# native-m/whitebox

Hardware: AMD Instinct MI355X
Metric: stereo fp32 frames/sec mixed (4096 tracks @ 512-frame blocks) (higher is better)
Workload: dtype f32

## Files before the change

whitebox_amd/csrc/wbx_mix.h:

```cpp
#pragma once
#include <hip/hip_runtime.h>
#include <hip/hip_ext.h>

#include <cstdlib>
#include <type_traits>

#include "wbx_dev.h"
#include "wbx_shape.h"

namespace wbx {

typedef float f4 __attribute__((ext_vector_type(4)));
typedef float f4u __attribute__((ext_vector_type(4), aligned(4)));

#define WBX_GLOBAL __attribute__((address_space(1)))
template <class T>
__device__ __forceinline__ const T WBX_GLOBAL* as_global(const void* p) {
  return (const T WBX_GLOBAL*)(uintptr_t)p;
}

__device__ __forceinline__ void store_f4_system(float* p, f4 v) {
  asm volatile("global_store_dwordx4 %0, %1, off sc0 sc1" : : "v"(p), "v"(v) : "memory");
}
__device__ __forceinline__ void store_u4_system(void* p, uint4 u) {
  const f4 v = {__uint_as_float(u.x), __uint_as_float(u.y), __uint_as_float(u.z), __uint_as_float(u.w)};
  asm volatile("global_store_dwordx4 %0, %1, off sc0 sc1" : : "v"(p), "v"(v) : "memory");
}

__device__ __forceinline__ float clampf(float x, float lo, float hi) {
  float m = x < hi ? x : hi;
  return m > lo ? m : lo;
}
__device__ __forceinline__ double clampd(double x, double lo, double hi) {
  double m = x < hi ? x : hi;
  return m > lo ? m : lo;
}

__device__ __forceinline__ float absmax4(f4 m) {
  float t;
  asm("v_max3_f32 %0, |%1|, |%2|, |%3|" : "=v"(t) : "v"(m.x), "v"(m.y), "v"(m.z));
  asm("v_max_f32_e64 %0, |%1|, %2" : "=v"(t) : "v"(m.w), "v"(t));
  return t;
}

__device__ __forceinline__ float sel_neg(int t, float a, float b) {
  const int m = t >> 31;
  float r;
  asm("v_bfi_b32 %0, %1, %2, %3" : "=v"(r) : "v"(m), "v"(a), "v"(b));
  return r;
}
template <int E>
__device__ __forceinline__ void taps(const f4& v, float w4, int k, float& sa, float& sb) {
  sa = v.x;
  sb = v.y;
  if (E >= 1) {
    sa = sel_neg(k - 1, sa, v.y);
    sb = sel_neg(k - 1, sb, v.z);
  }
  if (E >= 2) {
    sa = sel_neg(k - 2, sa, v.z);
    sb = sel_neg(k - 2, sb, v.w);
  }
  if (E >= 3) {
    sa = sel_neg(k - 3, sa, v.w);
    sb = sel_neg(k - 3, sb, w4);
  }
}

constexpr double kNarrowSpeed = 0.67;
template <int E>
__device__ __forceinline__ void taps_narrow(const f4& v, float w4, int k, float& sa, float& sb) {
  const int t = k - E;
  if (E == 1) {
    sa = sel_neg(t, v.x, v.y);
    sb = sel_neg(t, v.y, v.z);
  } else if (E == 2) {
    sa = sel_neg(t, v.y, v.z);
    sb = sel_neg(t, v.z, v.w);
  } else {
    sa = sel_neg(t, v.z, v.w);
    sb = sel_neg(t, v.w, w4);
  }
}

__device__ __forceinline__ float wave_max_lane63(float x) {
  uint32_t v = __float_as_uint(x);
#define WBX_DPP_MAX(ctrl, rmask)                                                                      \
  {                                                                                                  \
    const uint32_t o = (uint32_t)__builtin_amdgcn_update_dpp(0, (int)v, (ctrl), (rmask), 0xF, true);  \
    v = v > o ? v : o;                                                                               \
  }
  WBX_DPP_MAX(0xB1, 0xF)
  WBX_DPP_MAX(0x4E, 0xF)
  WBX_DPP_MAX(0x141, 0xF)
  WBX_DPP_MAX(0x140, 0xF)
  WBX_DPP_MAX(0x142, 0xA)
  WBX_DPP_MAX(0x143, 0xC)
#undef WBX_DPP_MAX
  return __uint_as_float(v);
}

__device__ __forceinline__ uint32_t wave_max_quad(uint32_t p0, uint32_t p1, uint32_t p2, uint32_t p3) {
  typedef unsigned int u2v __attribute__((ext_vector_type(2)));
  const u2v a = __builtin_amdgcn_permlane32_swap(p0, p1, false, false);
  const uint32_t m01 = a.x > a.y ? a.x : a.y;
  const u2v b = __builtin_amdgcn_permlane32_swap(p2, p3, false, false);
  const uint32_t m23 = b.x > b.y ? b.x : b.y;
  const u2v c = __builtin_amdgcn_permlane16_swap(m01, m23, false, false);
  uint32_t v = c.x > c.y ? c.x : c.y;
#define WBX_DPP_MAX(ctrl)                                                                         \
  {                                                                                               \
    const uint32_t o = (uint32_t)__builtin_amdgcn_update_dpp(0, (int)v, (ctrl), 0xF, 0xF, true);  \
    v = v > o ? v : o;                                                                            \
  }
  WBX_DPP_MAX(0xB1) WBX_DPP_MAX(0x4E) WBX_DPP_MAX(0x141) WBX_DPP_MAX(0x140)
#undef WBX_DPP_MAX
  return v;
}

__device__ __forceinline__ void wave_max_quad_halves(uint32_t p0, uint32_t p1, uint32_t p2, uint32_t p3, uint32_t& ch0,
                                                     uint32_t& ch1) {
  typedef unsigned int u2v __attribute__((ext_vector_type(2)));
  const u2v a = __builtin_amdgcn_permlane32_swap(p0, p1, false, false);
  const u2v b = __builtin_amdgcn_permlane32_swap(p2, p3, false, false);
  const u2v c0 = __builtin_amdgcn_permlane16_swap(a.x, b.x, false, false);
  const u2v c1 = __builtin_amdgcn_permlane16_swap(a.y, b.y, false, false);
  uint32_t v = c0.x > c0.y ? c0.x : c0.y, w = c1.x > c1.y ? c1.x : c1.y;
#define WBX_DPP_MAX(x, ctrl)                                                                      \
  {                                                                                               \
    const uint32_t o = (uint32_t)__builtin_amdgcn_update_dpp(0, (int)(x), (ctrl), 0xF, 0xF, true); \
    (x) = (x) > o ? (x) : o;                                                                      \
  }
  WBX_DPP_MAX(v, 0xB1) WBX_DPP_MAX(v, 0x4E) WBX_DPP_MAX(v, 0x141) WBX_DPP_MAX(v, 0x140)
  WBX_DPP_MAX(w, 0xB1) WBX_DPP_MAX(w, 0x4E) WBX_DPP_MAX(w, 0x141) WBX_DPP_MAX(w, 0x140)
#undef WBX_DPP_MAX
  ch0 = v;
  ch1 = w;
}

enum : int { MODE_U = 0, MODE_W = 1, MODE_I16 = 2, MODE_I32 = 3, MODE_MIXED = 4, MODE_WN = 5, MODE_G = 6, MODE_WI = 7, MODE_WIN = 8, MODE_MU = 9, MODE_MW = 10, MODE_MWN = 11,
             MODE_WNU = 12, MODE_WINU = 13 };

struct Win {
  f4 v;
  float w4;
};
template <int CL>
struct PreT {
  Win w[CL];
  int ix0;
  float fx0;
};
template <int CL>
struct PreGT {
  f4 v[CL], b[CL], fx;
};
template <int CL>
struct RowT {
  f4 c[CL];
};

template <int U, bool FULL, int FAM, int SB, int CW, int CL, int T, int X = 0>
__device__ __forceinline__ void mix_body(const MixArgs& a) {
  constexpr bool G = FAM == 1 || FAM == 3;
  constexpr bool STRIDE = FAM == 1;
  constexpr bool W16 = FAM >= 1;
  constexpr bool LEAN16 = FAM == 2;
  static_assert(SB == 1 || FULL, "sub-blocks need waves that stay inside one block");
  static_assert(CW == 1 || (CW == 2 && (SB == 4 || (SB == 1 && T == 64))), "two channels per wave: 128-frame stereo blocks, one block per wave");
  static_assert(CL == 1 || (CL == 2 && FULL && SB == 1 && CW == 1), "two channels per lane: stereo blocks of 4 * T frames");
  static_assert(T == 256 / CL || (CL == 2 && (T == 64 || T == 256)) || (CL == 1 && SB == 1 && (T == 64 || T == 128)), "lanes per workgroup");
  constexpr uint32_t kT = (uint32_t)T;
  constexpr bool XP = X != 0;
  static_assert(!XP || (SB > 1 && FULL), "masked rows in a packed instance");
  constexpr uint32_t kSt = XP ? (kStage >> (X == 1 ? 1 : 0)) / (SB == 4 ? 2u : 1u) : SB == 4 ? kStage / 2 : kT == 64u ? kStage / 2 : kStage;
  constexpr bool EXP = XP || (SB == 1 && FULL && (kSt == 128 || kT == 64u));
  constexpr uint32_t kMaxRows = EXP ? 2 * kSt : kSt;
  constexpr uint32_t kRecs = kMaxRows + 2 * U + 4;
  __shared__ __attribute__((aligned(16))) DTrackBlock s_tb[SB * kRecs];
  constexpr uint32_t kWaves = kT / 64u;
  constexpr uint32_t kPS = (CL == 2 && kWaves == 4u) ? 8u : 4u;
  __shared__ uint32_t s_pk[SB * kRecs * kPS];
  __shared__ uint32_t s_wc[kPS];
  __shared__ __attribute__((aligned(16))) DRow s_rows[EXP ? 2 * SB * kSt : 1];
  __shared__ uint32_t s_ord[EXP ? kSt : 1];
  __shared__ uint16_t s_map[EXP ? SB * 2 * kSt : 1];
  __shared__ uint16_t s_off[EXP ? SB * (kSt + 1) : 1];
  __shared__ uint32_t s_wpairs[3];
  __shared__ uint32_t s_hp[XP ? 8 : 1];
  __shared__ uint32_t s_tot[XP ? SB : 1];
  __shared__ int s_shape;

  const unsigned long long dbg_t0 = a.dbg_clock ? wall_clock64() : 0ull;
  uint32_t bx = blockIdx.x;
  if ((gridDim.x & 7u) == 0u) bx = (blockIdx.x & 7u) * (gridDim.x >> 3) + (blockIdx.x >> 3);
  const uint32_t g = blockIdx.y, tile = blockIdx.z;
  const uint32_t tid = threadIdx.x;
  const DGroup grp = a.groups[g];
  const uint32_t F = a.block_frames, C = a.channels, N = a.n_tracks;
  const uint32_t S4 = F >> 2;
  const uint32_t Lc = FULL ? a.lane_span : S4;
  const uint32_t sub = SB > 1 ? (uint32_t)__builtin_amdgcn_readfirstlane((int)(tid / (C * Lc))) : 0u;
  const uint32_t rb = sub * kRecs;
  const uint32_t b = bx * SB + sub;
  const bool bvalid = SB == 1 || b < a.n_blocks;
  const uint32_t slot = SB > 1 ? tid - sub * (C * Lc) : tile * kT + tid;
  const bool active = FULL ? true : (slot < C * S4);
  uint32_t c = active ? slot / Lc : 0u;
  if (FULL && CL == 1 && c >= C) c = C - 1u;
  if (FULL && CW == 1) c = __builtin_amdgcn_readfirstlane(c);
  const uint32_t jn = active ? slot - (slot / Lc) * Lc : 0u;
  if (CL == 2) c = 0u;
  const bool owns = FULL ? (jn < S4 && slot < C * Lc) : active;
  const uint32_t j0 = active ? (jn < S4 ? jn : S4 - 1u) * 4u : 0u;
  uint32_t span = 64u;
  if (!FULL) {
    span = S4 & (~S4 + 1u);
    span = span > 64u ? 64u : span;
  }
  const uint32_t lane = tid & 63u;
  const double j0d = (double)(int32_t)j0;

  using Pre = PreT<CL>;
  using PreG = PreGT<CL>;
  using Row = RowT<CL>;
  Row acc;
#pragma unroll
  for (int ch = 0; ch < CL; ch++) acc.c[ch] = f4{0.0f, 0.0f, 0.0f, 0.0f};
  if (a.init && g == 0u && owns && bvalid) {
#pragma unroll
    for (int ch = 0; ch < CL; ch++)
      acc.c[ch] = *reinterpret_cast<const f4*>(a.init + ((size_t)b * C + (CL == 2 ? (uint32_t)ch : c)) * F + j0);
  }

  const bool chain_in = a.chain != nullptr && (grp.flags & GROUP_CHAIN_IN) != 0u;
  const bool chain_out = a.chain != nullptr && (grp.flags & GROUP_CHAIN_OUT) != 0u;
  uint32_t* chain_word = a.chain ? a.chain + ((size_t)(blockIdx.x * a.tiles + tile) * a.n_groups + g) : nullptr;
  const uint32_t my_xcc = a.chain ? ((uint32_t)__builtin_amdgcn_s_getreg(63508) & 0xFu) + 1u : 0u;
  const uint32_t chain_tag = a.chain_epoch << 4;
  uint32_t chain_seen = 0u;
  if (chain_in && tid == 0u) chain_seen = __hip_atomic_load(chain_word - 1, __ATOMIC_RELAXED, __HIP_MEMORY_SCOPE_AGENT);

  const double jd1 = j0d + 1.0, jd2 = j0d + 2.0, jd3 = j0d + 3.0;
  const double us = a.uniform_speed;
  const double up0 = __dmul_rn(j0d, us), up1 = __dmul_rn(jd1, us), up2 = __dmul_rn(jd2, us), up3 = __dmul_rn(jd3, us);

  struct URec {
    const void* src[CL];
    double pos, speed;
    float gain, gc[CL];
    uint32_t kind, format;
    uint32_t d, n;
    bool partial;
  };
  auto load_urec = [&](uint32_t rec) {
    const int w = (int)reinterpret_cast<const uint32_t*>(&s_tb[rb + rec])[lane & 15u];
    auto rl = [&](uint32_t i) { return (uint32_t)__builtin_amdgcn_readlane(w, (int)i); };
    URec r;
    if (CW == 2) {
      const uint64_t s0 = ((uint64_t)rl(1) << 32) | rl(0), s1 = ((uint64_t)rl(3) << 32) | rl(2);
      r.src[0] = (const void*)(c ? s1 : s0);
      r.pos = __longlong_as_double((long long)(((uint64_t)rl(5) << 32) | rl(4)));
      r.speed = __longlong_as_double((long long)(((uint64_t)rl(7) << 32) | rl(6)));
      r.gain = __uint_as_float(rl(8));
      r.gc[0] = __uint_as_float(c ? rl(10) : rl(9));
      const uint32_t q11 = rl(11);
      r.kind = (q11 >> 8) & KIND_MASK;
      r.format = rl(13) & 0xFFu;
      if (EXP) {
        r.partial = ((q11 >> 15) & 1u) != 0u;
        r.d = 0u;
        r.n = F;
        if (r.partial) {
          r.d = q11 >> 16;
          r.n = rl(12) & 0xFFFFu;
        }
      }
      return r;
    }
    const uint32_t cs = FULL ? c : 0u;
#pragma unroll
    for (int ch = 0; ch < CL; ch++) {
      const uint32_t cc = CL == 2 ? (uint32_t)ch : cs;
      r.src[ch] = (const void*)(((uint64_t)rl(2u * cc + 1u) << 32) | rl(2u * cc));
      r.gc[ch] = __uint_as_float(rl(9u + cc));
    }
    r.pos = __longlong_as_double((long long)(((uint64_t)rl(5) << 32) | rl(4)));
    r.speed = __longlong_as_double((long long)(((uint64_t)rl(7) << 32) | rl(6)));
    r.gain = __uint_as_float(rl(8));
    const uint32_t q11 = rl(11);
    r.kind = (q11 >> 8) & KIND_MASK;
    r.format = rl(13) & 0xFFu;
    if (EXP) {
      r.partial = ((q11 >> 15) & 1u) != 0u;
      r.d = 0u;
      r.n = F;
      if (r.partial) {
        r.d = q11 >> 16;
        r.n = rl(12) & 0xFFFFu;
      }
    }
    return r;
  };
  const uint32_t wave_base = (uint32_t)__builtin_amdgcn_readfirstlane((int)j0);
  constexpr uint32_t kWF = CW == 2 ? 128u : 256u;
  const uint32_t wave_end = wave_base + kWF < F ? wave_base + kWF : F;
  auto call_frame = [&](uint32_t e, uint32_t d, uint32_t n) {
    const int x = (int)(j0 + e) - (int)d, hi = (int)n - 1;
    const int lo = x > 0 ? x : 0;
    return lo < hi ? lo : hi;
  };
  auto frame_mask = [&](uint32_t e, uint32_t d, uint32_t n) { return (uint32_t)0 - (uint32_t)((j0 + e - d) < n); };
  auto and_mask = [&](float v, uint32_t m) { return __uint_as_float(__float_as_uint(v) & m); };
  auto fast_part = [&](const URec& r) {
    return EXP && a.fast_partial != 0u && r.partial && __double2hiint(r.pos) >= 0x40100000;
  };
  auto part_cf0 = [&](const URec& r) {
    if (fast_part(r)) {
      const int x = (int)j0 - (int)r.d, hi = (int)r.n - 1;
      return ((int)j0 + 3 < (int)r.d) ? 0 : (x < hi ? x : hi);
    }
    return call_frame(0u, r.d, r.n);
  };

  auto row_f32 = [&](const f4& v, float cg, float gc) {
    f4 m;
    if (__float_as_uint(cg) == 0x3F800000u) {
      m.x = __fmul_rn(v.x, gc);
      m.y = __fmul_rn(v.y, gc);
      m.z = __fmul_rn(v.z, gc);
      m.w = __fmul_rn(v.w, gc);
    } else {
      m.x = __fmul_rn(__fmul_rn(v.x, cg), gc);
      m.y = __fmul_rn(__fmul_rn(v.y, cg), gc);
      m.z = __fmul_rn(__fmul_rn(v.z, cg), gc);
      m.w = __fmul_rn(__fmul_rn(v.w, cg), gc);
    }
    return m;
  };
  auto norm_i16 = [&](int lo, int hi) {
    const float norm = 1.0f / 32767.0f;
// ... 567 lines not shown
        const uint32_t fmt = (uint32_t)__builtin_amdgcn_readfirstlane((int)r.format);
        constexpr std::integral_constant<bool, MODE == MODE_MWN> narrow{};
        if (EXP && r.partial) {
          if (r.d >= wave_end || r.d + r.n <= wave_base) {
#pragma unroll
            for (int ch = 0; ch < CL; ch++) m.c[ch] = f4{0.0f, 0.0f, 0.0f, 0.0f};
          } else {
            Pre q = pre[u];
            const bool p16 = k == KIND_WINDOW_I16 || k == KIND_UNITY_I16;
            if (p16) {
#pragma unroll
              for (int ch = 0; ch < CL; ch++) q.w[ch].w4 = pre[u].w[ch].v.z;
            }
            m = partial_any(narrow, q, k, fmt, p16);
          }
        } else if (k == KIND_WINDOW_I16) {
          Pre q = pre[u];
#pragma unroll
          for (int ch = 0; ch < CL; ch++) q.w[ch].w4 = pre[u].w[ch].v.z;
          m = row_window16(narrow, std::false_type{}, q, r.pos, r.speed, cg, gc);
        } else if (k == KIND_WINDOW) {
          if (fmt == FMT_F32)
            m = row_window(narrow, pre[u], r.pos, r.speed, cg, gc);
          else
            m = row_window32(narrow, std::false_type{}, pre[u], fmt, r.pos, r.speed, cg, gc);
        } else if (k == KIND_UNITY_I16) {
          each_i16();
        } else if (k == KIND_UNITY_I32) {
          each_i32(fmt);
        } else {
          each_f32();
        }
      } else {
        const int k = MODE == MODE_U ? KIND_UNITY : MODE == MODE_I16 ? KIND_UNITY_I16 : MODE == MODE_I32 ? KIND_UNITY_I32
                                                  : __builtin_amdgcn_readfirstlane((int)r.kind);
        const uint32_t fmt = (MODE == MODE_I32 || MODE == MODE_MU) ? (uint32_t)__builtin_amdgcn_readfirstlane((int)r.format) : 0u;
        if (EXP && r.partial && !(r.d <= wave_base && r.d + r.n >= wave_end)) {
          if (r.d >= wave_end || r.d + r.n <= wave_base) {
#pragma unroll
            for (int ch = 0; ch < CL; ch++) m.c[ch] = f4{0.0f, 0.0f, 0.0f, 0.0f};
          } else if (fast_part(r)) {
            if (k == KIND_UNITY_I16)
              each_i16();
            else if (k == KIND_UNITY_I32)
              each_i32(fmt);
            else
              each_f32();
            mask_row(m, r.d, r.n);
          } else if (k == KIND_UNITY_I16) {
            each([&](const Win& w, float g) {
              return row_f32_masked(norm_i16(__float_as_int(w.v.x), __float_as_int(w.v.y)), r.d, r.n, cg, g);
            });
          } else if (k == KIND_UNITY_I32) {
            each([&](const Win& w, float g) { return row_f32_masked(norm_i32(w.v, fmt), r.d, r.n, cg, g); });
          } else {
            each([&](const Win& w, float g) { return row_f32_masked(w.v, r.d, r.n, cg, g); });
          }
        } else if (k == KIND_UNITY_I16) {
          each_i16();
        } else if (k == KIND_UNITY_I32) {
          each_i32(fmt);
        } else {
          each_f32();
        }
      }
      }
      add_row(m, pk[u]);
    }
  };

  auto pipeline = [&](auto mode, uint32_t cn) {
    constexpr int D = decltype(mode)::value == MODE_G ? 1 : U;
    constexpr int kIter = (2 * D) % 4 == 0 ? 2 * D : 4;
    std::conditional_t<decltype(mode)::value == MODE_G, PreG, Pre> pa[D], pb[D];
    issue(mode, 0, pa);
    for (uint32_t u0 = 0; u0 < cn; u0 += kIter) {
      float pk[kIter][CL];
#pragma unroll
      for (int h = 0; h < kIter; h += 2 * D) {
        issue(mode, u0 + h + D, pb);
        render(mode, u0 + h, pa, pk + h);
        issue(mode, u0 + h + 2 * D, pa);
        render(mode, u0 + h + D, pb, pk + h + D);
      }
#pragma unroll
      for (int ch = 0; ch < CL; ch++) {
        if (FULL) {
#pragma unroll
          for (int q = 0; q < kIter; q += 4) {
            const float quad[4] = {pk[q][ch], pk[q + 1][ch], pk[q + 2][ch], pk[q + 3][ch]};
            post_peak4(quad, u0 + q, ch);
          }
        } else {
#pragma unroll
          for (int q = 0; q < kIter; q++) post_peak(pk[q][ch], u0 + q, ch);
        }
      }
    }
  };

  auto mixed = [&](uint32_t cn) {
    for (uint32_t tl = 0; tl < cn; tl++) {
      const DTrackBlock& r = s_tb[rb + tl];
      const int k = __builtin_amdgcn_readfirstlane((int)(r.kind & KIND_MASK));
      const float cg = r.gain;
      const uint32_t off = (uint32_t)r.pos + j0;
      Row m;
      float gcs[CL];
      const void* srcs[CL];
#pragma unroll
      for (int ch = 0; ch < CL; ch++) {
        const uint32_t cc = CL == 2 ? (uint32_t)ch : c;
        gcs[ch] = r.g[cc];
        srcs[ch] = r.src[cc];
      }
      if (k == KIND_WINDOW) {
        Pre p;
        load_window(srcs, r.pos, __dmul_rn(j0d, r.speed), p);
        m = row_window(std::false_type{}, p, r.pos, r.speed, cg, gcs);
      } else if (W16 && (k == KIND_WINDOW_I16 || (EXP && LEAN16 && k == KIND_UNITY_I16 && (r.kind & KIND_PARTIAL)))) {
        Pre p;
        if (EXP && LEAN16 && (r.kind & KIND_PARTIAL)) {
          const uint32_t d = r.dst_start, n = r.len;
          load_window16(srcs, r.pos, __dmul_rn((double)call_frame(0u, d, n), r.speed), p);
          m = row_window16_masked(p, r.pos, r.speed, k != KIND_WINDOW_I16, d, n, cg, gcs);
        } else {
          load_window16(srcs, r.pos, __dmul_rn(j0d, r.speed), p);
          m = row_window16(std::false_type{}, std::false_type{}, p, r.pos, r.speed, cg, gcs);
        }
      } else {
#pragma unroll
        for (int ch = 0; ch < CL; ch++) {
          if (k == KIND_UNITY_I16) {
            typedef int i2u __attribute__((ext_vector_type(2), aligned(2)));
            i2u w = {0, 0};
            if (active) w = *reinterpret_cast<const i2u WBX_GLOBAL*>(as_global<short>(srcs[ch]) + off);
            m.c[ch] = row_i16(w.x, w.y, cg, gcs[ch]);
          } else {
            f4 v = {0.0f, 0.0f, 0.0f, 0.0f};
            if (active) v = *reinterpret_cast<const f4u WBX_GLOBAL*>(as_global<float>(srcs[ch]) + off);
            m.c[ch] = (k == KIND_UNITY_I32) ? row_i32(v, r.format, cg, gcs[ch]) : row_f32(v, cg, gcs[ch]);
          }
        }
      }
      float pk[CL];
      add_row(m, pk);
#pragma unroll
      for (int ch = 0; ch < CL; ch++) post_peak(pk[ch], tl, ch);
    }
  };

  uint32_t chunk0 = 0u, cn2 = 0u;
  int mode = MODE_U;
  for (uint32_t chunk_i = 0u; chunk0 < grp.count; chunk_i++) {
    const uint32_t left = grp.count - chunk0;
    const uint32_t cn = left < kSt ? left : kSt;
    cn2 = cn;
    __syncthreads();
    if (tid == 0u) s_shape = 0;
    if constexpr (XP) {
      constexpr uint32_t kHalves = kSt / 32u;
      DRow* rows_cur = s_rows + (chunk_i & 1u) * (SB * kSt);
      DRow* rows_nxt = s_rows + ((chunk_i & 1u) ^ 1u) * (SB * kSt);
      const uint32_t n0 = chunk0 + cn, nleft = grp.count - n0, ncn = nleft < kSt ? nleft : kSt;
      const uint32_t m0 = n0 + ncn, mleft = grp.count - m0, mcn = mleft < kSt ? mleft : kSt;
      uint32_t before = 0u;
      bool is_pair = false;
      const uint32_t psb = tid / kSt, pt = tid - psb * kSt;
      DRow nrow;
      nrow.pos = 0.0;
      nrow.tmpl = 0xFFFFFFFFu;
      nrow.flags = ROW_SILENT;
      uint32_t nord = 0u;
      if (tid < SB * kSt) {
        DRow row = nrow;
        const uint32_t bb = bx * SB + psb;
        const bool bval = bb < a.n_blocks;
        uint32_t o1 = 0u;
        if (chunk_i == 0u) {
          uint32_t o0 = 0u;
          if (pt < cn) o0 = a.order[grp.first + pt];
          if (pt < ncn) o1 = a.order[grp.first + n0 + pt];
          if (pt < cn && bval) row = a.rows[(size_t)bb * N + o0];
          *reinterpret_cast<uint4*>(&rows_cur[tid]) = *reinterpret_cast<const uint4*>(&row);
        } else {
          row = rows_cur[tid];
          o1 = s_ord[pt];
        }
        if (pt < ncn && bval) nrow = a.rows[(size_t)bb * N + o1];
        if (psb == 0u && pt < mcn) nord = a.order[grp.first + m0 + pt];
        is_pair = (row.flags & (ROW_PAIR | ROW_SILENT)) == ROW_PAIR;
        const unsigned long long half = (lane & 32u) ? 0xFFFFFFFF00000000ull : 0x00000000FFFFFFFFull;
        const unsigned long long bal = __ballot(is_pair) & half;
        before = (uint32_t)__popcll(bal & ((1ull << lane) - 1ull));
        if ((lane & 31u) == 0u) s_hp[tid >> 5] = (uint32_t)__popcll(bal);
      }
      __syncthreads();
      if (tid < SB * kSt) {
        uint32_t off = pt + before, total = cn;
#pragma unroll
        for (uint32_t h = 0; h < kHalves; h++) {
          const uint32_t n = s_hp[psb * kHalves + h];
          if (psb * kHalves + h < (tid >> 5)) off += n;
          total += n;
        }
        if (pt < cn) {
          s_off[psb * (kSt + 1u) + pt] = (uint16_t)off;
          s_map[psb * 2u * kSt + off] = (uint16_t)pt;
          if (is_pair) s_map[psb * 2u * kSt + off + 1u] = (uint16_t)(pt | 0x8000u);
        }
        if (pt == 0u) {
          s_off[psb * (kSt + 1u) + cn] = (uint16_t)total;
          s_tot[psb] = total;
        }
      }
      __syncthreads();
      cn2 = (uint32_t)__builtin_amdgcn_readfirstlane((int)s_tot[sub]);
      constexpr uint32_t kQ = (SB * kRecs * 4u + kT - 1u) / kT;
      uint4 wq[kQ];
      uint32_t tq = tid;
      asm volatile("" : "+v"(tq));
#pragma unroll
      for (uint32_t it = 0; it < kQ; it++) {
        const uint32_t i = tq + it * kT, sbq = i / (kRecs * 4u), r4 = i - sbq * (kRecs * 4u), rec = r4 >> 2, q = r4 & 3u;
        const bool in = sbq < (uint32_t)SB && rec < s_tot[sbq < (uint32_t)SB ? sbq : 0u];
        const uint32_t mp = s_map[in ? sbq * 2u * kSt + rec : 0u];
        const DRow row = rows_cur[(in ? sbq * kSt : 0u) + (mp & 0x7FFFu)];
        const bool live = in && !(row.flags & ROW_SILENT);
        wq[it] = reinterpret_cast<const uint4*>(a.tmpl + (live ? row.tmpl + (mp >> 15) : 0u))[q];
      }
#pragma unroll
      for (uint32_t it = 0; it < kQ; it++) {
        const uint32_t i = tq + it * kT, sbq = i / (kRecs * 4u), r4 = i - sbq * (kRecs * 4u), rec = r4 >> 2, q = r4 & 3u;
        if (i < SB * kRecs * 4u) {
          uint4 w = {0u, 0u, 0u, 0u};
          if (rec < s_tot[sbq]) {
            const uint32_t mp = s_map[sbq * 2u * kSt + rec];
            const DRow row = rows_cur[sbq * kSt + (mp & 0x7FFFu)];
            if (!(row.flags & ROW_SILENT)) {
              w = wq[it];
              if (q == 1u && (row.flags & ROW_POS)) {
                const uint2 pb = *reinterpret_cast<const uint2*>(&row.pos);
                w.x = pb.x;
                w.y = pb.y;
              }
            }
          }
          reinterpret_cast<uint4*>(s_tb)[i] = w;
        }
      }
      if (tid < SB * kSt) {
        *reinterpret_cast<uint4*>(&rows_nxt[tid]) = *reinterpret_cast<const uint4*>(&nrow);
        if (psb == 0u) s_ord[pt] = nord;
      }
    } else if constexpr (EXP) {
      DRow* rows_cur = s_rows + (chunk_i & 1u) * kSt;
      DRow* rows_nxt = s_rows + ((chunk_i & 1u) ^ 1u) * kSt;
      const uint32_t n0 = chunk0 + cn, nleft = grp.count - n0, ncn = nleft < kSt ? nleft : kSt;
      const uint32_t m0 = n0 + ncn, mleft = grp.count - m0, mcn = mleft < kSt ? mleft : kSt;
      uint32_t before = 0u;
      bool is_pair = false;
      DRow nrow;
      nrow.pos = 0.0;
      nrow.tmpl = 0xFFFFFFFFu;
      nrow.flags = ROW_SILENT;
      uint32_t nord = 0u;
      if (tid < kSt) {
        DRow row = nrow;
        uint32_t o1 = 0u;
        if (chunk_i == 0u) {
          uint32_t o0 = 0u;
          if (tid < cn) o0 = a.order[grp.first + tid];
          if (tid < ncn) o1 = a.order[grp.first + n0 + tid];
          if (tid < cn) row = a.rows[(size_t)bx * N + o0];
        } else {
          row = rows_cur[tid];
          o1 = s_ord[tid];
        }
        if (tid < ncn) nrow = a.rows[(size_t)bx * N + o1];
        if (tid < mcn) nord = a.order[grp.first + m0 + tid];
        if (chunk_i == 0u) *reinterpret_cast<uint4*>(&rows_cur[tid]) = *reinterpret_cast<const uint4*>(&row);
        is_pair = (row.flags & (ROW_PAIR | ROW_SILENT)) == ROW_PAIR;
        const unsigned long long bal = __ballot(is_pair);
        before = (uint32_t)__popcll(bal & ((1ull << lane) - 1ull));
        if (lane == 0u) s_wpairs[tid >> 6] = (uint32_t)__popcll(bal);
        if (kSt <= 64u && tid == 0u) s_wpairs[1] = 0u;
      }
      __syncthreads();
      if (tid < cn) {
        const uint32_t off = tid + before + (tid >= 64u ? s_wpairs[0] : 0u);
        s_off[tid] = (uint16_t)off;
        s_map[off] = (uint16_t)tid;
        if (is_pair) s_map[off + 1u] = (uint16_t)(tid | 0x8000u);
      }
      if (tid == 0u) {
        const uint32_t total = cn + s_wpairs[0] + s_wpairs[1];
        s_off[cn] = (uint16_t)total;
        s_wpairs[2] = total;
      }
      __syncthreads();
      cn2 = (uint32_t)__builtin_amdgcn_readfirstlane((int)s_wpairs[2]);
      constexpr uint32_t kQ = (kRecs * 4u + kT - 1u) / kT;
      const uint32_t nq = (cn2 * 4u + kT - 1u) / kT;
      uint4 wq[kQ];
      uint32_t tq = tid;
      asm volatile("" : "+v"(tq));
#pragma unroll
      for (uint32_t it = 0; it < kQ; it++) {
        wq[it] = uint4{0u, 0u, 0u, 0u};
        if (it < nq) {
          const uint32_t i = tq + it * kT, rec = i >> 2, q = i & 3u;
          const bool in = rec < cn2;
          const uint32_t mp = s_map[in ? rec : 0u];
          const DRow row = rows_cur[mp & 0x7FFFu];
          const bool live = in && !(row.flags & ROW_SILENT);
          wq[it] = reinterpret_cast<const uint4*>(a.tmpl + (live ? row.tmpl + (mp >> 15) : 0u))[q];
        }
      }
#pragma unroll
      for (uint32_t it = 0; it < kQ; it++) {
        const uint32_t i = tq + it * kT, rec = i >> 2, q = i & 3u;
        if (i < kRecs * 4u) {
          uint4 w = {0u, 0u, 0u, 0u};
          if (it < nq && rec < cn2) {
            const uint32_t mp = s_map[rec];
            const DRow row = rows_cur[mp & 0x7FFFu];
            if (!(row.flags & ROW_SILENT)) {
              w = wq[it];
              if (q == 1u && (row.flags & ROW_POS)) {
                const uint2 pb = *reinterpret_cast<const uint2*>(&row.pos);
                w.x = pb.x;
                w.y = pb.y;
              }
            }
          }
          reinterpret_cast<uint4*>(s_tb)[i] = w;
        }
      }
      if (tid < kSt) {
        *reinterpret_cast<uint4*>(&rows_nxt[tid]) = *reinterpret_cast<const uint4*>(&nrow);
        s_ord[tid] = nord;
      }
    } else {
    for (uint32_t i = tid; i < SB * kRecs * 4u; i += kT) {
      const uint32_t sb = SB > 1 ? i / (kRecs * 4u) : 0u;
      const uint32_t rec = (i - sb * kRecs * 4u) >> 2, q = i & 3u;
      const uint32_t bb = bx * SB + sb;
      uint4 w = {0u, 0u, 0u, 0u};
      if (rec < cn && (SB == 1 || bb < a.n_blocks)) {
        const uint32_t track = a.order[grp.first + chunk0 + rec];
        const DRow row = a.rows[(size_t)bb * N + track];
        if (!(row.flags & ROW_SILENT)) {
          w = reinterpret_cast<const uint4*>(a.tmpl + row.tmpl)[q];
          if (q == 1u && (row.flags & ROW_POS)) {
            const uint2 pb = *reinterpret_cast<const uint2*>(&row.pos);
            w.x = pb.x;
            w.y = pb.y;
          }
        }
      }
      reinterpret_cast<uint4*>(s_tb)[i] = w;
    }
    }
    for (uint32_t i = tid; i < SB * kRecs * kPS; i += kT) s_pk[i] = 0u;
    if (FULL && lane == 0u) {
      if (CL == 2) {
        s_wc[wave] = 0u;
        s_wc[kWaves + wave] = 1u;
        if (2u * kWaves < kPS && wave == 0u) {
          s_wc[2] = 0xFFFFFFFFu;
          s_wc[3] = 0xFFFFFFFFu;
        }
      } else {
        s_wc[wave] = sub * C + c;
      }
    }
    __syncthreads();
    int shape = 0;
    for (uint32_t i0 = tid; i0 < SB * (XP ? kMaxRows : cn2); i0 += kT) {
      if (XP && i0 % kMaxRows >= s_tot[XP ? i0 / kMaxRows : 0u]) continue;
      const uint32_t i = XP ? (i0 / kMaxRows) * kRecs + i0 % kMaxRows : SB > 1 ? (i0 / cn2) * kRecs + i0 % cn2 : i0;
      const int k = s_tb[i].kind & KIND_MASK;
      shape |= k == KIND_UNITY ? 1 : k == KIND_WINDOW ? (s_tb[i].format == FMT_F32 ? 2 : 128) : k == KIND_UNITY_I16 ? 4 : k == KIND_UNITY_I32 ? 8
               : k == KIND_STRIDE ? 64 : k == KIND_WINDOW_I16 ? 32 : 0;
      if ((k == KIND_WINDOW || k == KIND_WINDOW_I16) && !(s_tb[i].speed >= kNarrowSpeed)) shape |= 16;
    }
    if (shape) atomicOr(&s_shape, shape);
    __syncthreads();
    const int shapes = __builtin_amdgcn_readfirstlane(s_shape);
    const int has_f32 = shapes & 3, has_win = shapes & 2, has_i16 = shapes & 4, has_i32 = shapes & 8, has_wide = shapes & 16;
    const int has_stride = STRIDE ? (shapes & 64) : 0;
    const int has_win16 = W16 ? (shapes & 32) : 0;
    const int has_win32 = G ? (shapes & 128) : 0;
    if (LEAN16) {
      if (has_win16)
        mode = (!has_f32 && !has_i32) ? (has_wide ? MODE_WI : us > 0.0 ? MODE_WINU : MODE_WIN) : MODE_MIXED;
      else if (has_i16)
        mode = (!has_f32 && !has_i32) ? MODE_I16 : (has_win || has_i32) ? MODE_MIXED : MODE_MU;
      else
        mode = (has_win || has_i32) ? MODE_MIXED : MODE_U;
    } else if (has_stride) {
      mode = MODE_G;
    } else if (has_win16) {
      mode = (!has_f32 && !has_i32 && !has_win32) ? (has_wide ? MODE_WI : us > 0.0 ? MODE_WINU : MODE_WIN) : (has_wide ? MODE_MW : MODE_MWN);
    } else if (has_i16) {
      mode = (has_win32 || (G && has_win)) ? (has_wide ? MODE_MW : MODE_MWN)
             : (!has_i32 && !has_f32) ? MODE_I16 : has_win ? MODE_MIXED : MODE_MU;
    } else if (has_win || has_win32) {
      mode = (G || !has_i32) ? (has_wide ? MODE_W : us > 0.0 ? MODE_WNU : MODE_WN) : MODE_MIXED;
    } else {
      mode = !has_i32 ? MODE_U : !has_f32 ? MODE_I32 : MODE_MU;
    }
    for (uint32_t i = tid; i < SB * kRecs; i += kT) {
      DTrackBlock& r = s_tb[i];
      if ((SB > 1 ? i % kRecs : i) >= (XP ? s_tot[XP ? i / kRecs : 0u] : cn2) || (r.kind & KIND_MASK) == KIND_SILENT || (r.kind & KIND_MASK) == KIND_GENERIC) {
        r.src[0] = a.zero_page;
        r.src[1] = a.zero_page;
        r.pos = 0.0;
        r.speed = 1.0;
        r.gain = 0.0f;
        r.g[0] = 0.0f;
        r.g[1] = 0.0f;
        r.dst_start = 0;
        r.len = (uint16_t)F;
        const bool m16 = mode == MODE_I16 || mode == MODE_WI || mode == MODE_WIN || mode == MODE_WINU;
        r.format = m16 ? FMT_I16 : mode == MODE_I32 ? FMT_I32 : FMT_F32;
        r.kind = m16 ? KIND_UNITY_I16 : mode == MODE_I32 ? KIND_UNITY_I32 : KIND_UNITY;
      }
    }
    __syncthreads();

    if (chain_in && chunk_i == 0u) {
      if (tid == 0u) {
        uint32_t spins = 0u;
        while ((chain_seen & ~0xFu) != chain_tag && spins < 400000u) {
          __builtin_amdgcn_s_sleep(8);
          chain_seen = __hip_atomic_load(chain_word - 1, __ATOMIC_RELAXED, __HIP_MEMORY_SCOPE_AGENT);
          spins++;
        }
        const bool chain_ok = (chain_seen & ~0xFu) == chain_tag;
        if (!chain_ok && a.chain_status) {
          atomicOr(a.chain_status, 32u);
          atomicOr(a.chain_sticky, 32u);
        }
        if (chain_ok && (chain_seen & 0xFu) != my_xcc && a.chain_status) {
          atomicOr(a.chain_status, 64u);
          atomicOr(a.chain_sticky, 64u);
        }
      }
      __syncthreads();
      if (owns && bvalid) {
#pragma unroll
        for (int ch = 0; ch < CL; ch++) {
          const uint32_t* src = reinterpret_cast<const uint32_t*>(
              a.partial + (((size_t)b * a.n_groups + (g - 1u)) * C + (CL == 2 ? (uint32_t)ch : c)) * F + j0);
          acc.c[ch].x = __uint_as_float(__hip_atomic_load(src + 0, __ATOMIC_RELAXED, __HIP_MEMORY_SCOPE_AGENT));
          acc.c[ch].y = __uint_as_float(__hip_atomic_load(src + 1, __ATOMIC_RELAXED, __HIP_MEMORY_SCOPE_AGENT));
          acc.c[ch].z = __uint_as_float(__hip_atomic_load(src + 2, __ATOMIC_RELAXED, __HIP_MEMORY_SCOPE_AGENT));
          acc.c[ch].w = __uint_as_float(__hip_atomic_load(src + 3, __ATOMIC_RELAXED, __HIP_MEMORY_SCOPE_AGENT));
        }
      }
    }

    switch (mode) {
      case MODE_U: pipeline(std::integral_constant<int, MODE_U>{}, cn2); break;
      case MODE_W:
        if constexpr (!LEAN16) pipeline(std::integral_constant<int, MODE_W>{}, cn2);
        break;
      case MODE_WN:
        if constexpr (!LEAN16) pipeline(std::integral_constant<int, MODE_WN>{}, cn2);
        break;
      case MODE_WNU:
        if constexpr (!LEAN16) pipeline(std::integral_constant<int, MODE_WNU>{}, cn2);
        break;
      case MODE_G:
        if constexpr (STRIDE) pipeline(std::integral_constant<int, MODE_G>{}, cn2);
        break;
      case MODE_WI:
        if constexpr (W16) pipeline(std::integral_constant<int, MODE_WI>{}, cn2);
        break;
      case MODE_WIN:
        if constexpr (W16) pipeline(std::integral_constant<int, MODE_WIN>{}, cn2);
        break;
      case MODE_WINU:
        if constexpr (W16) pipeline(std::integral_constant<int, MODE_WINU>{}, cn2);
        break;
      case MODE_MU: pipeline(std::integral_constant<int, MODE_MU>{}, cn2); break;
      case MODE_MW:
        if constexpr (G) pipeline(std::integral_constant<int, MODE_MW>{}, cn2);
        break;
      case MODE_MWN:
        if constexpr (G) pipeline(std::integral_constant<int, MODE_MWN>{}, cn2);
        break;
      case MODE_I16: pipeline(std::integral_constant<int, MODE_I16>{}, cn2); break;
      case MODE_I32:
        if constexpr (!LEAN16) pipeline(std::integral_constant<int, MODE_I32>{}, cn2);
        break;
      default: mixed(cn2); break;
    }

    __syncthreads();
    for (uint32_t i0 = tid; i0 < SB * cn * C; i0 += kT) {
      const uint32_t sb = SB > 1 ? i0 / (cn * C) : 0u;
      const uint32_t i = i0 - sb * cn * C;
      const uint32_t rec = i / C, ch = i - rec * C;
      const uint32_t bb = bx * SB + sb;
      if (SB > 1 && bb >= a.n_blocks) continue;
      const uint32_t track = a.order[grp.first + chunk0 + rec];
      uint32_t* dst = reinterpret_cast<uint32_t*>(a.peaks) + ((size_t)bb * N + track) * C + ch;
      uint32_t pk = 0u;
      if (FULL && CW == 2) {
        const uint32_t r0 = EXP ? s_off[sb * (kSt + 1u) + rec] : rec;
        const uint32_t r1 = EXP ? s_off[sb * (kSt + 1u) + rec + 1u] : rec + 1u;
        for (uint32_t rr = r0; rr < r1; rr++) {
          const uint32_t v = s_pk[(sb * kRecs + rr) * kPS + ch];
          pk = pk > v ? pk : v;
        }
      } else if (FULL) {
        const uint32_t r0 = EXP ? s_off[sb * (kSt + 1u) + rec] : rec;
        const uint32_t r1 = EXP ? s_off[sb * (kSt + 1u) + rec + 1u] : rec + 1u;
        for (uint32_t rr = r0; rr < r1; rr++) {
          const uint32_t* slots = &s_pk[(sb * kRecs + rr) * kPS];
#pragma unroll
          for (uint32_t w = 0; w < kPS; w++)
            if (s_wc[w] == sb * C + ch) pk = pk > slots[w] ? pk : slots[w];
        }
      } else {
        pk = s_pk[rec * 2u + ch];
      }
      if (a.tiles == 1u)
        *dst = pk;
      else
        atomicMax(dst, pk);
      if (a.levels && pk != 0u) atomicMax(a.levels + (size_t)track * C + ch, pk);
    }
    chunk0 += cn;
  }

  if (a.dbg_clock && tid == 0u) {
    const uint32_t wg = blockIdx.x + gridDim.x * (blockIdx.y + gridDim.y * blockIdx.z);
    a.dbg_clock[4u * wg] = dbg_t0;
    a.dbg_clock[4u * wg + 1u] = wall_clock64();
    a.dbg_clock[4u * wg + 2u] = (unsigned long long)(uint32_t)__builtin_amdgcn_s_getreg(63492);
    a.dbg_clock[4u * wg + 3u] = (unsigned long long)(uint32_t)__builtin_amdgcn_s_getreg(63508);
  }
  if (a.fused_master) {
    if (a.fused_status_dst && blockIdx.x == 0u && tid < 4u) {
      const uint32_t queued = a.fused_status_src[2];
      if (a.partial_through)
        __hip_atomic_store(a.fused_status_dst + tid, a.fused_status_src[tid], __ATOMIC_RELAXED, __HIP_MEMORY_SCOPE_SYSTEM);
      else
        a.fused_status_dst[tid] = a.fused_status_src[tid];
      if (a.fused_zero_status && queued == 0u) a.fused_status_src[tid] = 0u;
    }
    if (owns && bvalid) {
#pragma unroll
      for (int ch = 0; ch < CL; ch++) {
        f4 m = acc.c[ch];
        m.x = __fadd_rn(0.0f, m.x);
        m.y = __fadd_rn(0.0f, m.y);
        m.z = __fadd_rn(0.0f, m.z);
        m.w = __fadd_rn(0.0f, m.w);
        if (a.fused_clamp) {
          m.x = m.x > 1.0f ? 1.0f : (m.x < -1.0f ? -1.0f : m.x);
          m.y = m.y > 1.0f ? 1.0f : (m.y < -1.0f ? -1.0f : m.y);
          m.z = m.z > 1.0f ? 1.0f : (m.z < -1.0f ? -1.0f : m.z);
          m.w = m.w > 1.0f ? 1.0f : (m.w < -1.0f ? -1.0f : m.w);
        }
        float* mo = a.fused_master + ((size_t)b * C + (CL == 2 ? (uint32_t)ch : c)) * F + j0;
        if (a.partial_through)
          store_f4_system(mo, m);
        else
          *reinterpret_cast<f4*>(mo) = m;
      }
    }
  } else if (owns && bvalid) {
#pragma unroll
    for (int ch = 0; ch < CL; ch++) {
      float* out = a.partial + (((size_t)b * a.n_groups + g) * C + (CL == 2 ? (uint32_t)ch : c)) * F + j0;
      if (a.partial_through) {
        uint32_t* o = reinterpret_cast<uint32_t*>(out);
        __hip_atomic_store(o + 0, __float_as_uint(acc.c[ch].x), __ATOMIC_RELAXED, __HIP_MEMORY_SCOPE_AGENT);
        __hip_atomic_store(o + 1, __float_as_uint(acc.c[ch].y), __ATOMIC_RELAXED, __HIP_MEMORY_SCOPE_AGENT);
        __hip_atomic_store(o + 2, __float_as_uint(acc.c[ch].z), __ATOMIC_RELAXED, __HIP_MEMORY_SCOPE_AGENT);
        __hip_atomic_store(o + 3, __float_as_uint(acc.c[ch].w), __ATOMIC_RELAXED, __HIP_MEMORY_SCOPE_AGENT);
      } else {
        *reinterpret_cast<f4*>(out) = acc.c[ch];
      }
    }
  }
  if (chain_out) {
    __builtin_amdgcn_s_waitcnt(0);
    __syncthreads();
    if (tid == 0u) __hip_atomic_store(chain_word, chain_tag | my_xcc, __ATOMIC_RELAXED, __HIP_MEMORY_SCOPE_AGENT);
  }
}

template <int U, bool FULL, int W, int FAM, int SB, int CW = 1, int CL = 1, int T = 256 / CL>
__global__ __launch_bounds__(T, W) void mix_kernel(MixArgs a) {
  mix_body<U, FULL, FAM, SB, CW, CL, T>(a);
}
template <int U, int W, int FAM, int SB, int CW, int X>
__global__ __launch_bounds__(256, W) void mix_kernel_x(MixArgs a) {
  mix_body<U, true, FAM, SB, CW, 1, 256, X>(a);
}

struct MixEntry {
  MixInstance inst;
  const char* name;
  void (*launch)(const MixArgs& a, dim3 grid, hipStream_t s, hipEvent_t t0, hipEvent_t t1);
};
#define WBX_MIX(U, FULL, W, FAM, SB, CW, CL, T)                                                                \
  {MixInstance::mix(U, FULL, W, FAM, SB, CW, CL, T),                                                           \
// ... 32 lines not shown
```

Before: 185.0 million.

## Fold shape detection and zero-row patching into staging pass, trim barriers

Computes the per-record shape bitmask and the zero-row flags while the track records are staged, in registers, using quad DPP broadcasts and a wave OR-reduction. This removes the separate LDS re-scan and its barrier. Zero-row patching now rewrites only flagged quads, the window-pair offset map skips its extra barrier when no pairs exist, s_pk clearing is skipped in FULL mode, and chained partial loads use vectorised dwordx4 agent-scope loads instead of scalar atomics. The cost is more register state and extra DPP/ALU work per staged quad, plus inline asm with explicit waitcnt.

```diff
diff --git a/whitebox_amd/csrc/wbx_mix.h b/whitebox_amd/csrc/wbx_mix.h
--- a/whitebox_amd/csrc/wbx_mix.h
+++ b/whitebox_amd/csrc/wbx_mix.h
@@ -25,6 +25,23 @@
 __device__ __forceinline__ void store_u4_system(void* p, uint4 u) {
   const f4 v = {__uint_as_float(u.x), __uint_as_float(u.y), __uint_as_float(u.z), __uint_as_float(u.w)};
   asm volatile("global_store_dwordx4 %0, %1, off sc0 sc1" : : "v"(p), "v"(v) : "memory");
+}
+
+__device__ __forceinline__ f4 load_f4_agent(const float* p) {
+  f4 v;
+  asm volatile("global_load_dwordx4 %0, %1, off sc1\n\ts_waitcnt vmcnt(0)" : "=&v"(v) : "v"(p) : "memory");
+  return v;
+}
+__device__ __forceinline__ void load_f4x2_agent(const float* p0, const float* p1, f4& v0, f4& v1) {
+  asm volatile("global_load_dwordx4 %0, %2, off sc1\n\tglobal_load_dwordx4 %1, %3, off sc1\n\ts_waitcnt vmcnt(0)"
+               : "=&v"(v0), "=&v"(v1)
+               : "v"(p0), "v"(p1)
+               : "memory");
+}
+
+template <int Q>
+__device__ __forceinline__ uint32_t quad_bcast(uint32_t v) {
+  return (uint32_t)__builtin_amdgcn_update_dpp(0, (int)v, Q * 0x55, 0xF, 0xF, true);
 }
 
 __device__ __forceinline__ float clampf(float x, float lo, float hi) {
@@ -98,6 +115,36 @@
   WBX_DPP_MAX(0x143, 0xC)
 #undef WBX_DPP_MAX
   return __uint_as_float(v);
+}
+
+__device__ __forceinline__ uint32_t wave_or_lane63(uint32_t v) {
+#define WBX_DPP_OR(ctrl, rmask) v |= (uint32_t)__builtin_amdgcn_update_dpp(0, (int)v, (ctrl), (rmask), 0xF, true);
+  WBX_DPP_OR(0xB1, 0xF)
+  WBX_DPP_OR(0x4E, 0xF)
+  WBX_DPP_OR(0x141, 0xF)
+  WBX_DPP_OR(0x140, 0xF)
+  WBX_DPP_OR(0x142, 0xA)
+  WBX_DPP_OR(0x143, 0xC)
+#undef WBX_DPP_OR
+  return v;
+}
+
+__device__ __forceinline__ int staged_record_shape(const uint4& w, bool& zero_row) {
+  const int k = (int)((quad_bcast<2>(w.w) >> 8) & KIND_MASK);
+  const uint32_t format = quad_bcast<3>(w.y) & 0xFFu;
+  const double speed = __hiloint2double((int)quad_bcast<1>(w.w), (int)quad_bcast<1>(w.z));
+  zero_row = k == KIND_SILENT || k == KIND_GENERIC;
+  int shape = k == KIND_UNITY ? 1 : k == KIND_WINDOW ? (format == FMT_F32 ? 2 : 128) : k == KIND_UNITY_I16 ? 4 : k == KIND_UNITY_I32 ? 8
+              : k == KIND_STRIDE ? 64 : k == KIND_WINDOW_I16 ? 32 : 0;
+  if ((k == KIND_WINDOW || k == KIND_WINDOW_I16) && !(speed >= kNarrowSpeed)) shape |= 16;
+  return shape;
+}
+__device__ __forceinline__ uint4 stage_zero_quad(uint4 w, uint32_t q, const void* zero_page, uint32_t F, uint32_t kind, uint32_t format) {
+  const uint32_t zlo = (uint32_t)(uintptr_t)zero_page, zhi = (uint32_t)((uintptr_t)zero_page >> 32);
+  if (q == 0u) return uint4{zlo, zhi, zlo, zhi};
+  if (q == 1u) return uint4{0u, 0u, 0u, 0x3FF00000u};
+  if (q == 2u) return uint4{0u, 0u, 0u, (w.w & 0xFFu) | (kind << 8)};
+  return uint4{(w.x & 0xFFFF0000u) | (F & 0xFFFFu), (w.y & 0xFFFFFF00u) | format, w.z, w.w};
 }
 
 __device__ __forceinline__ uint32_t wave_max_quad(uint32_t p0, uint32_t p1, uint32_t p2, uint32_t p3) {
@@ -186,7 +233,7 @@
   __shared__ uint32_t s_ord[EXP ? kSt : 1];
   __shared__ uint16_t s_map[EXP ? SB * 2 * kSt : 1];
   __shared__ uint16_t s_off[EXP ? SB * (kSt + 1) : 1];
-  __shared__ uint32_t s_wpairs[3];
+  __shared__ uint32_t s_wpairs[2];
   __shared__ uint32_t s_hp[XP ? 8 : 1];
   __shared__ uint32_t s_tot[XP ? SB : 1];
   __shared__ int s_shape;
@@ -1060,12 +1107,14 @@
 
   uint32_t chunk0 = 0u, cn2 = 0u;
   int mode = MODE_U;
+  if (tid == 0u) s_shape = 0;
   for (uint32_t chunk_i = 0u; chunk0 < grp.count; chunk_i++) {
     const uint32_t left = grp.count - chunk0;
     const uint32_t cn = left < kSt ? left : kSt;
     cn2 = cn;
     __syncthreads();
-    if (tid == 0u) s_shape = 0;
+    int shape = 0;
+    uint32_t zero_quads = 0u;
     if constexpr (XP) {
       constexpr uint32_t kHalves = kSt / 32u;
       DRow* rows_cur = s_rows + (chunk_i & 1u) * (SB * kSt);
@@ -1140,21 +1189,24 @@
 #pragma unroll
       for (uint32_t it = 0; it < kQ; it++) {
         const uint32_t i = tq + it * kT, sbq = i / (kRecs * 4u), r4 = i - sbq * (kRecs * 4u), rec = r4 >> 2, q = r4 & 3u;
-        if (i < SB * kRecs * 4u) {
-          uint4 w = {0u, 0u, 0u, 0u};
-          if (rec < s_tot[sbq]) {
-            const uint32_t mp = s_map[sbq * 2u * kSt + rec];
-            const DRow row = rows_cur[sbq * kSt + (mp & 0x7FFFu)];
-            if (!(row.flags & ROW_SILENT)) {
-              w = wq[it];
-              if (q == 1u && (row.flags & ROW_POS)) {
-                const uint2 pb = *reinterpret_cast<const uint2*>(&row.pos);
-                w.x = pb.x;
-                w.y = pb.y;
-              }
+        uint4 w = {0u, 0u, 0u, 0u};
+        if (i < SB * kRecs * 4u && rec < s_tot[sbq]) {
+          const uint32_t mp = s_map[sbq * 2u * kSt + rec];
+          const DRow row = rows_cur[sbq * kSt + (mp & 0x7FFFu)];
+          if (!(row.flags & ROW_SILENT)) {
+            w = wq[it];
+            if (q == 1u && (row.flags & ROW_POS)) {
+              const uint2 pb = *reinterpret_cast<const uint2*>(&row.pos);
+              w.x = pb.x;
+              w.y = pb.y;
             }
           }
+        }
+        bool zero_row;
+        shape |= staged_record_shape(w, zero_row);
+        if (i < SB * kRecs * 4u) {
           reinterpret_cast<uint4*>(s_tb)[i] = w;
+          zero_quads |= (zero_row ? 1u : 0u) << it;
         }
       }
       if (tid < SB * kSt) {
@@ -1193,21 +1245,25 @@
         before = (uint32_t)__popcll(bal & ((1ull << lane) - 1ull));
         if (lane == 0u) s_wpairs[tid >> 6] = (uint32_t)__popcll(bal);
         if (kSt <= 64u && tid == 0u) s_wpairs[1] = 0u;
+        if (tid < cn) {
+          s_off[tid] = (uint16_t)tid;
+          s_map[tid] = (uint16_t)tid;
+        }
+        if (tid == 0u) s_off[cn] = (uint16_t)cn;
       }
       __syncthreads();
-      if (tid < cn) {
-        const uint32_t off = tid + before + (tid >= 64u ? s_wpairs[0] : 0u);
-        s_off[tid] = (uint16_t)off;
-        s_map[off] = (uint16_t)tid;
-        if (is_pair) s_map[off + 1u] = (uint16_t)(tid | 0x8000u);
-      }
-      if (tid == 0u) {
-        const uint32_t total = cn + s_wpairs[0] + s_wpairs[1];
-        s_off[cn] = (uint16_t)total;
-        s_wpairs[2] = total;
-      }
-      __syncthreads();
-      cn2 = (uint32_t)__builtin_amdgcn_readfirstlane((int)s_wpairs[2]);
+      const uint32_t pairs = (uint32_t)__builtin_amdgcn_readfirstlane((int)(s_wpairs[0] + s_wpairs[1]));
+      if (pairs != 0u) {
+        if (tid < cn) {
+          const uint32_t off = tid + before + (tid >= 64u ? s_wpairs[0] : 0u);
+          s_off[tid] = (uint16_t)off;
+          s_map[off] = (uint16_t)tid;
+          if (is_pair) s_map[off + 1u] = (uint16_t)(tid | 0x8000u);
+        }
+        if (tid == 0u) s_off[cn] = (uint16_t)(cn + pairs);
+        __syncthreads();
+      }
+      cn2 = cn + pairs;
       constexpr uint32_t kQ = (kRecs * 4u + kT - 1u) / kT;
       const uint32_t nq = (cn2 * 4u + kT - 1u) / kT;
       uint4 wq[kQ];
@@ -1228,21 +1284,24 @@
 #pragma unroll
       for (uint32_t it = 0; it < kQ; it++) {
         const uint32_t i = tq + it * kT, rec = i >> 2, q = i & 3u;
-        if (i < kRecs * 4u) {
-          uint4 w = {0u, 0u, 0u, 0u};
-          if (it < nq && rec < cn2) {
-            const uint32_t mp = s_map[rec];
-            const DRow row = rows_cur[mp & 0x7FFFu];
-            if (!(row.flags & ROW_SILENT)) {
-              w = wq[it];
-              if (q == 1u && (row.flags & ROW_POS)) {
-                const uint2 pb = *reinterpret_cast<const uint2*>(&row.pos);
-                w.x = pb.x;
-                w.y = pb.y;
-              }
+        uint4 w = {0u, 0u, 0u, 0u};
+        if (it < nq && rec < cn2) {
+          const uint32_t mp = s_map[rec];
+          const DRow row = rows_cur[mp & 0x7FFFu];
+          if (!(row.flags & ROW_SILENT)) {
+            w = wq[it];
+            if (q == 1u && (row.flags & ROW_POS)) {
+              const uint2 pb = *reinterpret_cast<const uint2*>(&row.pos);
+              w.x = pb.x;
+              w.y = pb.y;
             }
           }
+        }
+        bool zero_row = true;
+        if (it < nq) shape |= staged_record_shape(w, zero_row);
+        if (i < kRecs * 4u) {
           reinterpret_cast<uint4*>(s_tb)[i] = w;
+          zero_quads |= (zero_row ? 1u : 0u) << it;
         }
       }
       if (tid < kSt) {
@@ -1250,7 +1309,8 @@
         s_ord[tid] = nord;
       }
     } else {
-    for (uint32_t i = tid; i < SB * kRecs * 4u; i += kT) {
+    uint32_t it = 0u;
+    for (uint32_t i = tid; i < SB * kRecs * 4u; i += kT, it++) {
       const uint32_t sb = SB > 1 ? i / (kRecs * 4u) : 0u;
       const uint32_t rec = (i - sb * kRecs * 4u) >> 2, q = i & 3u;
       const uint32_t bb = bx * SB + sb;
@@ -1268,9 +1328,17 @@
         }
       }
       reinterpret_cast<uint4*>(s_tb)[i] = w;
-    }
-    }
-    for (uint32_t i = tid; i < SB * kRecs * kPS; i += kT) s_pk[i] = 0u;
+      bool zero_row;
+      shape |= staged_record_shape(w, zero_row);
+      zero_quads |= (zero_row ? 1u : 0u) << it;
+    }
+    }
+    {
+      const uint32_t wave_shape = wave_or_lane63((uint32_t)shape);
+      if (lane == 63u && wave_shape != 0u) atomicOr(&s_shape, (int)wave_shape);
+    }
+    if (!FULL)
+      for (uint32_t i = tid; i < SB * kRecs * kPS; i += kT) s_pk[i] = 0u;
     if (FULL && lane == 0u) {
       if (CL == 2) {
         s_wc[wave] = 0u;
@@ -1281,19 +1349,10 @@
         }
       } else {
         s_wc[wave] = sub * C + c;
-      }
-    }
-    __syncthreads();
-    int shape = 0;
-    for (uint32_t i0 = tid; i0 < SB * (XP ? kMaxRows : cn2); i0 += kT) {
-      if (XP && i0 % kMaxRows >= s_tot[XP ? i0 / kMaxRows : 0u]) continue;
-      const uint32_t i = XP ? (i0 / kMaxRows) * kRecs + i0 % kMaxRows : SB > 1 ? (i0 / cn2) * kRecs + i0 % cn2 : i0;
-      const int k = s_tb[i].kind & KIND_MASK;
-      shape |= k == KIND_UNITY ? 1 : k == KIND_WINDOW ? (s_tb[i].format == FMT_F32 ? 2 : 128) : k == KIND_UNITY_I16 ? 4 : k == KIND_UNITY_I32 ? 8
-               : k == KIND_STRIDE ? 64 : k == KIND_WINDOW_I16 ? 32 : 0;
-      if ((k == KIND_WINDOW || k == KIND_WINDOW_I16) && !(s_tb[i].speed >= kNarrowSpeed)) shape |= 16;
-    }
-    if (shape) atomicOr(&s_shape, shape);
+        if (kWaves < kPS && wave == 0u)
+          for (uint32_t w = kWaves; w < kPS; w++) s_wc[w] = 0xFFFFFFFFu;
+      }
+    }
     __syncthreads();
     const int shapes = __builtin_amdgcn_readfirstlane(s_shape);
     const int has_f32 = shapes & 3, has_win = shapes & 2, has_i16 = shapes & 4, has_i32 = shapes & 8, has_wide = shapes & 16;
@@ -1319,24 +1378,21 @@
     } else {
       mode = !has_i32 ? MODE_U : !has_f32 ? MODE_I32 : MODE_MU;
     }
-    for (uint32_t i = tid; i < SB * kRecs; i += kT) {
-      DTrackBlock& r = s_tb[i];
-      if ((SB > 1 ? i % kRecs : i) >= (XP ? s_tot[XP ? i / kRecs : 0u] : cn2) || (r.kind & KIND_MASK) == KIND_SILENT || (r.kind & KIND_MASK) == KIND_GENERIC) {
-        r.src[0] = a.zero_page;
-        r.src[1] = a.zero_page;
-        r.pos = 0.0;
-        r.speed = 1.0;
-        r.gain = 0.0f;
-        r.g[0] = 0.0f;
-        r.g[1] = 0.0f;
-        r.dst_start = 0;
-        r.len = (uint16_t)F;
-        const bool m16 = mode == MODE_I16 || mode == MODE_WI || mode == MODE_WIN || mode == MODE_WINU;
-        r.format = m16 ? FMT_I16 : mode == MODE_I32 ? FMT_I32 : FMT_F32;
-        r.kind = m16 ? KIND_UNITY_I16 : mode == MODE_I32 ? KIND_UNITY_I32 : KIND_UNITY;
+    {
+      const bool m16 = mode == MODE_I16 || mode == MODE_WI || mode == MODE_WIN || mode == MODE_WINU;
+      const uint32_t zfmt = m16 ? FMT_I16 : mode == MODE_I32 ? FMT_I32 : FMT_F32;
+      const uint32_t zkind = m16 ? KIND_UNITY_I16 : mode == MODE_I32 ? KIND_UNITY_I32 : KIND_UNITY;
+      constexpr uint32_t kZ = (SB * kRecs * 4u + kT - 1u) / kT;
+#pragma unroll
+      for (uint32_t it = 0; it < kZ; it++) {
+        if (zero_quads & (1u << it)) {
+          uint4* qp = reinterpret_cast<uint4*>(s_tb) + (tid + it * kT);
+          *qp = stage_zero_quad(*qp, tid & 3u, a.zero_page, F, zkind, zfmt);
+        }
       }
     }
     __syncthreads();
+    if (tid == 0u) s_shape = 0;
 
     if (chain_in && chunk_i == 0u) {
       if (tid == 0u) {
@@ -1358,15 +1414,11 @@
       }
       __syncthreads();
       if (owns && bvalid) {
-#pragma unroll
-        for (int ch = 0; ch < CL; ch++) {
-          const uint32_t* src = reinterpret_cast<const uint32_t*>(
-              a.partial + (((size_t)b * a.n_groups + (g - 1u)) * C + (CL == 2 ? (uint32_t)ch : c)) * F + j0);
-          acc.c[ch].x = __uint_as_float(__hip_atomic_load(src + 0, __ATOMIC_RELAXED, __HIP_MEMORY_SCOPE_AGENT));
-          acc.c[ch].y = __uint_as_float(__hip_atomic_load(src + 1, __ATOMIC_RELAXED, __HIP_MEMORY_SCOPE_AGENT));
-          acc.c[ch].z = __uint_as_float(__hip_atomic_load(src + 2, __ATOMIC_RELAXED, __HIP_MEMORY_SCOPE_AGENT));
-          acc.c[ch].w = __uint_as_float(__hip_atomic_load(src + 3, __ATOMIC_RELAXED, __HIP_MEMORY_SCOPE_AGENT));
-        }
+        const float* src = a.partial + (((size_t)b * a.n_groups + (g - 1u)) * C + (CL == 2 ? 0u : c)) * F + j0;
+        if constexpr (CL == 2)
+          load_f4x2_agent(src, src + F, acc.c[0], acc.c[CL - 1]);
+        else
+          acc.c[0] = load_f4_agent(src);
       }
     }
 
```

Result: no change. 183.4 million (-0.9%).
